# yinnhao/TAIR

Measured on AMD Instinct MI355X. Metric: restored Mpix/s @50-step SpacedSampler, 512² bf16; PSNR Δ vs ref ≤0.05 dB, higher is better.
Workload: dtype bf16; 1 GPU; configs[1]: 512x512 restoration, 50-step SpacedSampler, ControlLDM bf16, 1 tile(s)/GPU, hipGraph-replayed step, VAE decode included; tiles_per_gpu=1, micro_batch=1, global_batch=1, latent=64x64, sampling_steps=50, vae=HIP decoder, split-bf16 MFMA (fp32-accurate), parallelism=dp1 (tile-sharded replicas; RCCL all-gather of decoded tiles)

## Files before the change

### include/tair_kernels.h

```cpp
#ifndef TAIR_KERNELS_H
#define TAIR_KERNELS_H

#include <stdint.h>

#ifdef __cplusplus
extern "C" {
#endif

#define TAIR_A_DENSE 0
#define TAIR_A_CONV3 1
#define TAIR_A_CONV3_S2 2
#define TAIR_A_CONV3_UP 3
#define TAIR_A_CONV3_SMALLC 4

typedef struct {
  int M, N, K, amode;
  const void* A; int lda; int C; int Bn, H, W, Ho, Wo;
  const void* X; int ldx; int Kx;
  const void* Wt; int ldw;
  float alpha; int scale_bias; int act;
  const float* bias;
  const float* emb; int ld_emb; const int* emb_row; int rows_per_b;
  const void* res; int ld_res;
  void* out; int ldo; int out_f32;
  float* partial; int64_t partial_cap;
  int force_bm, force_bn, force_splits;
  int force_stages;
  int* tile_sem; int sem_cap;
  int out_split; int res_lo;
  double* st_acc; int st_rs, st_cg, st_G, st_coff, st_hw;
  int out_lo; int x_wrap;
  int probe;
  int f8; const float* row_scale; const float* col_scale;
  int s2_shift;
  const double* gn_st; int gn_rs; int gn_G; float gn_eps; const float* gn_gamma; const float* gn_beta; int gn_silu;
  unsigned long long* stamps;
  double* rst; const double* lnst; const float* lncs; float ln_c; float ln_eps;
} tair_gemm_desc;

int tair_k_gemm(const tair_gemm_desc* d, void* stream);
int tair_fault_count(int reset, int* count);
int tair_k_gemm_desc_bytes(void);
int tair_k_gemm_plan(const tair_gemm_desc* d, int* bm, int* bn, int* splits, int* kern);
int tair_k_attention_plan(int B, int H, int Sq, int Skv, int64_t ws_bytes, int* qsets, int* splits, int* kv_split);
int tair_k_attention(const void* q, int ldq, const void* k, int ldk, const void* v, int ldv, void* o, int ldo,
                     int B, int H, int Sq, int Skv, int kv_bstride, float scale, void* stream);
int tair_k_attention_ex(const void* q, int ldq, const void* k, int ldk, const void* v, int ldv, void* o, int ldo,
                        int B, int H, int Sq, int Skv, int kv_bstride, float scale, void* ws, int64_t ws_bytes,
                        int force_qsets, int force_splits, void* stream);
int tair_k_attention_tk(const void* q, int ldq, const void* k, int ldk, const void* v, int ldv, void* o, int ldo,
                        int B, int H, int Sq, int Skv, int kv_bstride, float scale, void* ws, int64_t ws_bytes,
                        int* tickets, int tickets_cap, int force_qsets, int force_splits, void* stream);
int tair_k_groupnorm(const void* x, int ldx, int B, int HW, int C, int G, float eps, const float* gamma,
                     const float* beta, int silu, void* y, int ldy, float* ss, float* ws, void* stream);
int tair_k_groupnorm_ex(const void* x, int ldx, int B, int HW, int C, int G, float eps, const float* gamma,
                        const float* beta, int silu, void* y, int ldy, float* ss, float* ws, int* tickets,
                        void* stream);
int tair_k_layernorm(const void* x, int T, int C, const float* gamma, const float* beta, float eps, void* y,
                     void* stream);
int tair_k_layernorm_fp8(const void* x, int T, int C, const float* gamma, const float* beta, float eps, void* y8,
                         int ld8, float* s8, void* stream);
int tair_k_quant_rows_fp8(const void* w, int rows, int K, int ldw, void* q, int ldq, float* scale, void* stream);
int tair_k_quant_rows_fp8_ex(const void* w, int rows, int K, int Kx, int ldw, const float* a, void* q, int ldq, int k8,
                             float* scale, void* stream);
int tair_k_gn_apply_fp8(const void* x, int ldx, int x_lo, int B, int HW, int C, int G, float eps, const float* gamma,
                        const float* beta, int silu, const double* st, int st_rs, const float* inv8, void* y8, int ld8,
// ... 34 lines not shown
```

### tair_amd/_lib.py

```python
from __future__ import annotations

import ctypes
import os
from typing import Optional

_HERE = os.path.dirname(os.path.abspath(__file__))
LIB_PATH = os.path.join(_HERE, "libtair_cldm.so")

TAIR_DTYPE_F32 = 0
TAIR_DTYPE_BF16 = 1
TAIR_DTYPE_FP8 = 2


class TairError(RuntimeError):
    pass


class CldmCfg(ctypes.Structure):
    _fields_ = [
        ("model_channels", ctypes.c_int),
        ("num_levels", ctypes.c_int),
        ("channel_mult", ctypes.c_int * 8),
        ("num_res_blocks", ctypes.c_int),
        ("num_attention_ds", ctypes.c_int),
# ... 86 lines not shown
    "tair_cldm_param_count": (_I, [_P, ctypes.POINTER(_I)]),
    "tair_cldm_param_info": (_I, [_P, _I, ctypes.POINTER(ctypes.c_char_p), ctypes.POINTER(ctypes.c_int64),
                                  ctypes.POINTER(_I)]),
    "tair_cldm_load_param": (_I, [_P, ctypes.c_char_p, _P, _I, ctypes.POINTER(ctypes.c_int64), _I]),
    "tair_cldm_finalize": (_I, [_P]),
    "tair_cldm_forward": (_I, [_P, ctypes.POINTER(CldmIO), _P]),
    "tair_sampler_set_schedule": (_I, [_P, _I, ctypes.POINTER(ctypes.c_int64), ctypes.POINTER(ctypes.c_float)]),
    "tair_sampler_prepare": (_I, [_P, ctypes.POINTER(SamplerIO), _P]),
    "tair_sampler_prepare_guided": (_I, [_P, ctypes.POINTER(SamplerIO), ctypes.POINTER(GuidanceIO), _P]),
    "tair_sampler_set_context": (_I, [_P, _P, _I, _P]),
    "tair_sampler_run": (_I, [_P, _I, _I, _P]),
    "tair_sampler_get_x": (_I, [_P, _P, _P, _P]),
    "tair_sampler_get_v": (_I, [_P, _P, _P]),
    "tair_profile_enable": (_I, [_P, _I]),
    "tair_profile_read": (_I, [_P, _I, ctypes.POINTER(ctypes.c_double), ctypes.POINTER(_I),
                               ctypes.POINTER(ctypes.c_double)]),
    "tair_cldm_flops": (_I, [_P, _I, ctypes.POINTER(ctypes.c_double)]),
    "tair_profile_dump": (_I, [_P, ctypes.c_char_p]),
    "tair_k_gemm": (_I, [ctypes.POINTER(GemmDesc), _P]),
    "tair_k_gemm_desc_bytes": (_I, []),
    "tair_fault_count": (_I, [_I, ctypes.POINTER(_I)]),
    "tair_k_gemm_plan": (_I, [ctypes.POINTER(GemmDesc), ctypes.POINTER(_I), ctypes.POINTER(_I), ctypes.POINTER(_I),
                              ctypes.POINTER(_I)]),
    "tair_k_attention_plan": (_I, [_I, _I, _I, _I, ctypes.c_int64, ctypes.POINTER(_I), ctypes.POINTER(_I),
                                   ctypes.POINTER(_I)]),
    "tair_k_attention": (_I, [_P, _I, _P, _I, _P, _I, _P, _I, _I, _I, _I, _I, _I, ctypes.c_float, _P]),
    "tair_k_attention_ex": (_I, [_P, _I, _P, _I, _P, _I, _P, _I, _I, _I, _I, _I, _I, ctypes.c_float, _P,
                                 ctypes.c_int64, _I, _I, _P]),
    "tair_k_attention_tk": (_I, [_P, _I, _P, _I, _P, _I, _P, _I, _I, _I, _I, _I, _I, ctypes.c_float, _P,
                                 ctypes.c_int64, _P, _I, _I, _I, _P]),
    "tair_k_groupnorm": (_I, [_P, _I, _I, _I, _I, _I, ctypes.c_float, _P, _P, _I, _P, _I, _P, _P, _P]),
    "tair_k_groupnorm_ex": (_I, [_P, _I, _I, _I, _I, _I, ctypes.c_float, _P, _P, _I, _P, _I, _P, _P, _P, _P]),
    "tair_k_layernorm": (_I, [_P, _I, _I, _P, _P, ctypes.c_float, _P, _P]),
    "tair_k_layernorm_fp8": (_I, [_P, _I, _I, _P, _P, ctypes.c_float, _P, _I, _P, _P]),
    "tair_k_quant_rows_fp8": (_I, [_P, _I, _I, _I, _P, _I, _P, _P]),
    "tair_k_geglu": (_I, [_P, _I, _I, _P, _P]),
    "tair_k_compose_ffpout": (_I, [_P, _P, _P, _P, _I, _P, _I, _P]),
    "tair_k_quant_rows_fp8_ex": (_I, [_P, _I, _I, _I, _I, _P, _P, _I, _I, _P, _P]),
    "tair_k_gn_apply_fp8": (_I, [_P, _I, _I, _I, _I, _I, _I, ctypes.c_float, _P, _P, _I, _P, _I, _P, _P, _I, _P]),
    "tair_k_sampler_step": (_I, [_P, _P, _P, _P, _P, _P, _P, _I, _I, _P, _P, _I, _I, _I, _P]),
    "tair_k_merge_overlap": (_I, [_P, _I, _I, _I, _I, _I, _I, _P, _I, _I, _I, _P, _P]),
    "tair_k_stitch_peers": (_I, [_P, _I, _I, _I, _I, _I, _I, _I, _I, _I, _I, _P, _I, _I, _I, _P, _P]),
    "tair_ipc_get_handle": (_I, [_P, _P, ctypes.POINTER(ctypes.c_ulonglong)]),
    "tair_ipc_open": (_I, [_P, ctypes.POINTER(ctypes.c_void_p)]),
    "tair_ipc_close": (_I, [_P]),
    "tair_k_gn_apply_stats": (_I, [_P, _I, _I, _I, _I, _I, _I, ctypes.c_float, _P, _P, _I, _P, _I, _P, _I, _I, _P]),
# ... 62 lines not shown
```

### tair_amd/csrc/gemm.hip

```cpp
#include <algorithm>

#include "gemm_kern.h"
#ifndef TAIR_BATCH_XCD
#define TAIR_BATCH_XCD 1
#endif

namespace tair {
namespace {

template <int S>
__global__ __launch_bounds__(256) void splitk_reduce_kernel(const GemmGroup P, int RB, int CB4) {
  const EpiArgs p = epi_args(P.g[blockIdx.z]);
  __shared__ double red[4 * STAT_NG];
  const int n4 = (p.N + 3) / 4;
  const size_t slab = (size_t)p.M * p.N;
  const bool vec = (p.N & 3) == 0;
  const bool stats = p.st[0].acc != nullptr;
  const int rpp = 256 / CB4;
  const int t = threadIdx.x;
  const int r0 = blockIdx.x * RB;
  const int c4_0 = blockIdx.y * CB4;
  if (stats) {
    for (int i = t; i < 4 * STAT_NG; i += 256) red[i] = 0.0;
    __syncthreads();
// ... 87 lines not shown
  TAIR_HIP_CHECK((gemm_set_attrs<A_DENSE, SET_SMALL>()));
  TAIR_HIP_CHECK((gemm_set_attrs<A_DENSE, SET_BIG>()));
  TAIR_HIP_CHECK((gemm_set_attrs<A_CONV3, SET_SMALL>()));
  TAIR_HIP_CHECK((gemm_set_attrs<A_CONV3, SET_BIG>()));
  TAIR_HIP_CHECK((gemm_set_attrs<A_CONV3_S2, SET_SMALL>()));
  TAIR_HIP_CHECK((gemm_set_attrs<A_CONV3_S2, SET_BIG>()));
  TAIR_HIP_CHECK((gemm_set_attrs<A_CONV3_UP, SET_SMALL>()));
  TAIR_HIP_CHECK((gemm_set_attrs<A_CONV3_UP, SET_BIG>()));
  TAIR_HIP_CHECK((gemm_set_attrs<A_CONV3_SMALLC, SET_REG>()));
  TAIR_HIP_CHECK((gemm_set_attrs<A_DENSE, SET_RING>()));
  TAIR_HIP_CHECK((gemm_set_attrs<A_CONV3, SET_RING>()));
  TAIR_HIP_CHECK((gemm_set_attrs<A_CONV3_S2, SET_RING>()));
  TAIR_HIP_CHECK((gemm_set_attrs<A_CONV3_UP, SET_RING>()));
  TAIR_HIP_CHECK((gemm_set_attrs<A_DENSE, SET_PHASE>()));
  TAIR_HIP_CHECK((gemm_set_attrs<A_DENSE, SET_SHALLOW>()));
  TAIR_HIP_CHECK((gemm_set_attrs<A_CONV3, SET_PHASE>()));
  TAIR_HIP_CHECK((gemm_set_attrs<A_CONV3_S2, SET_PHASE>()));
  TAIR_HIP_CHECK((gemm_set_attrs<A_CONV3_UP, SET_PHASE>()));
  TAIR_HIP_CHECK(set_attrs_f8<A_DENSE>());
  TAIR_HIP_CHECK((gemm_set_attrs<A_CONV3, SET_F8>()));
  TAIR_HIP_CHECK((gemm_set_attrs<A_CONV3, SET_HALO>()));
  TAIR_HIP_CHECK((gemm_set_attrs<A_DENSE, SET_DEEP>()));
  TAIR_HIP_CHECK((gemm_set_attrs<A_CONV3, SET_DEEP>()));
  done = true;
  return hipSuccess;
}

namespace {
hipError_t launch_set(int amode, GemmGroup& P, int n, int bm, int bn, int splits, int kern, hipStream_t s) {
  if (kern == GEMM_KERN_SHALLOW) return gemm_set_launch<A_DENSE, SET_SHALLOW>(P, n, bm, bn, splits, s);
  if (kern == GEMM_KERN_HALO) return gemm_set_launch<A_CONV3, SET_HALO>(P, n, bm, bn, splits, s);
  if (kern == GEMM_KERN_DEEP)
    return amode == A_DENSE ? gemm_set_launch<A_DENSE, SET_DEEP>(P, n, bm, bn, splits, s)
                            : gemm_set_launch<A_CONV3, SET_DEEP>(P, n, bm, bn, splits, s);
  if (kern == GEMM_KERN_PHASE) {
    switch (amode) {
      case A_DENSE: return gemm_set_launch<A_DENSE, SET_PHASE>(P, n, bm, bn, splits, s);
      case A_CONV3: return gemm_set_launch<A_CONV3, SET_PHASE>(P, n, bm, bn, splits, s);
      case A_CONV3_S2: return gemm_set_launch<A_CONV3_S2, SET_PHASE>(P, n, bm, bn, splits, s);
      default: return gemm_set_launch<A_CONV3_UP, SET_PHASE>(P, n, bm, bn, splits, s);
    }
  }
  if (bm < 0) {
    switch (amode) {
      case A_DENSE: return gemm_set_launch<A_DENSE, SET_RING>(P, n, -bm, bn, splits, s);
      case A_CONV3: return gemm_set_launch<A_CONV3, SET_RING>(P, n, -bm, bn, splits, s);
      case A_CONV3_S2: return gemm_set_launch<A_CONV3_S2, SET_RING>(P, n, -bm, bn, splits, s);
      default: return gemm_set_launch<A_CONV3_UP, SET_RING>(P, n, -bm, bn, splits, s);
    }
  }
  const bool big = gemm_tile_is_big(bm, bn);
  switch (amode) {
    case A_DENSE:
      return big ? gemm_set_launch<A_DENSE, SET_BIG>(P, n, bm, bn, splits, s)
                 : gemm_set_launch<A_DENSE, SET_SMALL>(P, n, bm, bn, splits, s);
    case A_CONV3:
      return big ? gemm_set_launch<A_CONV3, SET_BIG>(P, n, bm, bn, splits, s)
// ... 155 lines not shown
  *splits = s;
}

bool gemm_rowstats_ok(const GemmArgs& a) {
  static double probe_rst[2];
  GemmArgs b = a;
  if (!b.rst) b.rst = probe_rst;
  int bm, bn, s, kern;
  gemm_plan(b, &bm, &bn, &s, &kern);
  if (a.force_bm) bm = a.force_bm;
  return kern != GEMM_KERN_PHASE && (bm < 0 ? -bm : bm) <= 128 && !a.out_f32 && !a.out_split && a.act != 2 &&
         !a.st[0].acc;
}

size_t gemm_partial_elems(const GemmArgs& a) {
  int bm, bn, s;
  gemm_plan(a, &bm, &bn, &s);
  return s > 1 ? (size_t)s * a.M * a.N : 0;
}

static bool g_skip_reduce = false;
void gemm_set_skip_reduce(bool on) { g_skip_reduce = on; }

static int ink_smax() {
  static int v = -1;
  if (v < 0) {
    const char* e = getenv("TAIR_INK_SMAX");
    v = e ? atoi(e) : 3;
    if (v > INK_SMAX_BUILT) v = INK_SMAX_BUILT;
  }
  return v;
}

namespace {
thread_local bool g_gemm_dry = false;
thread_local int g_dry_plan[4];
thread_local bool g_gn_halo_only = false;
size_t plan_lds(int kern, int bm, int bn, int W, bool halo_s2) {
  if (kern == GEMM_KERN_HALO) {
    const int hrp = W == 64 ? (bn == 64 ? 448 : 400) : W == 32 ? (bn == 128 ? 384 : 344) : (bn == 128 ? 384 : 328);
    const int st = bn == 64 ? 4 : halo_s2 ? 2 : 3;
    return (size_t)2 * hrp * 128 + (size_t)st * bn * 128;
  }
  const int st = kern == GEMM_KERN_SHALLOW ? 2 : (bm == 128 && bn == 320) || (bm == 256 && bn >= 256) ? 2 : 3;
  return (size_t)st * (bm + bn) * 128;
}
bool deep_built(int bm, int bn, int st) {
  return bm == 64 && ((bn == 64 && (st == 4 || st == 5 || st == 6 || st == 8)) || (bn == 128 && st >= 4 && st <= 6));
}
}

bool gemm_gn_ok(const GemmArgs& a) {
  g_gemm_dry = g_gn_halo_only = true;
  const hipError_t e = gemm_grouped(&a, 1, nullptr);
  g_gemm_dry = g_gn_halo_only = false;
  return e == hipSuccess;
}

hipError_t gemm_plan_query(const GemmArgs& a, int* bm, int* bn, int* splits, int* kern, int lanes) {
  GemmArgs g[MAX_GROUP];
  const int n = lanes < 1 ? 1 : lanes > MAX_GROUP ? MAX_GROUP : lanes;
  for (int i = 0; i < n; ++i) g[i] = a;
  g_gemm_dry = true;
  const hipError_t e = gemm_grouped(g, n, nullptr);
  g_gemm_dry = false;
  *bm = g_dry_plan[0];
  *bn = g_dry_plan[1];
  *splits = g_dry_plan[2];
// ... 60 lines not shown
    return hipErrorInvalidValue;
  }
  if (a.lnst && (!a.lncs || a.amode != A_DENSE || a.Kx || a.f8 || !(a.ln_c > 0.f) || a.rst || a.st[0].acc ||
                 (a.N & 7))) {
    set_error("gemm: a folded LayerNorm takes a dense bf16 GEMM with column sums and 1/C");
    return hipErrorInvalidValue;
  }
  for (int i = 1; i < n; ++i)
    if ((args[i].rst != nullptr) != (a.rst != nullptr) || (args[i].lnst != nullptr) != (a.lnst != nullptr)) {
      set_error("gemm: grouped GEMMs must share the LayerNorm roles");
      return hipErrorInvalidValue;
    }
  int bm, bn, splits, kern;
  gemm_plan(a, &bm, &bn, &splits, &kern, n);
  if (a.force_bm) bm = a.force_bm;
  if (a.force_bn) bn = a.force_bn;
  if (a.force_splits) splits = a.force_splits;
  if (splits < 1 || splits > 16) {
    set_error("gemm: %d K splits (1..16)", splits);
    return hipErrorInvalidValue;
  }
  int tile_stages = 0;
  if (a.force_bm || a.force_stages)
    kern = a.force_stages >= 100 ? GEMM_KERN_DEEP
           : a.force_stages == 9 ? GEMM_KERN_HALO
           : a.force_stages >= 4 ? GEMM_KERN_PHASE : a.force_stages == 2 ? GEMM_KERN_SHALLOW : GEMM_KERN_TILE;
  if (kern == GEMM_KERN_DEEP) {
    tile_stages = a.force_stages - 100;
    if (a.f8 || (a.amode != A_DENSE && a.amode != A_CONV3) || !deep_built(bm, bn, tile_stages) || a.gn_st) {
      set_error("gemm: deep-ring tile %dx%d with %d stages not built (bf16 dense / stride-1 conv only)", bm, bn,
                tile_stages);
      return hipErrorInvalidValue;
    }
  }
  if (kern == GEMM_KERN_HALO && (!conv_halo_ok(a) || !halo_tile_built(a.W, bm, bn))) {
    set_error("gemm: halo tiles take bf16 stride-1 3x3 convs over 16/32/64-wide images, tile %dx%d not built "
              "for width %d", bm, bn, a.W);
    return hipErrorInvalidValue;
  }
  if (kern == GEMM_KERN_SHALLOW && (a.amode != A_DENSE || bm != 64 || (bn != 64 && bn != 128) || splits > 1)) {
    set_error("gemm: the 2-stage tiles are dense 64x64 / 64x128 without split-K (got %dx%d, mode %d, %d splits)", bm,
              bn, a.amode, splits);
    return hipErrorInvalidValue;
  }
  if (kern == GEMM_KERN_PHASE) splits = 1;
  if (kern == GEMM_KERN_PHASE && (a.amode == A_CONV3_SMALLC || bm != 256 || (bn != 256 && bn != 320))) {
    set_error("gemm: the 4-phase kernel takes 256x256 / 256x320 tiles (got %dx%d, mode %d)", bm, bn, a.amode);
    return hipErrorInvalidValue;
  }
  int st_hw = 0;
  for (int i = 0; i < n; ++i) {
    const GemmArgs& b = args[i];
    for (int k = 0; k < 2; ++k) {
      const StatTgt& t = b.st[k];
      if (!t.acc) continue;
      const bool groups_ok = t.cg >= 8 || (t.cg % 4 == 0 && t.c_off % 4 == 0);
// ... 47 lines not shown
      bm = 128;
      bn = a.amode == A_DENSE ? 256 : 320;
    }
    if (kern == GEMM_KERN_TILE && bm == 256 && bn != 128) bm = 128;
    if (kern == GEMM_KERN_TILE && bm == 128 && bn == 160) bn = 128;
    if (kern != GEMM_KERN_HALO)
      while (bm > 64 && a.rows_per_b % bm) bm >>= 1;
    const bool pipe_tile = kern == GEMM_KERN_SHALLOW || (bm == 128 && (bn == 256 || bn == 320)) ||
                           (bm == 256 && bn == 128);
    if (bm < 0 || (kern != GEMM_KERN_TILE && kern != GEMM_KERN_SHALLOW && kern != GEMM_KERN_HALO) ||
        (kern != GEMM_KERN_HALO && (a.rows_per_b % bm || !gemm_tile_built(a.amode, bm, bn) || !pipe_tile))) {
      set_error("gemm: no GroupNorm-on-load plan (tile %dx%d, kernel %d)", bm, bn, kern);
      return hipErrorInvalidValue;
    }
  }
  for (int i = 0; i < n; ++i) {
    const GemmArgs& b = args[i];
    while (splits > 1 && (b.partial == nullptr || (size_t)splits * b.M * b.N > b.partial_cap)) --splits;
  }
  {
    const int units = kern == GEMM_KERN_HALO ? a.C / 64 : (a.K + a.Kx) / (bm < 0 ? 32 : BK);
    while (splits > 1 && (long)(splits - 1) * cdiv(units, splits) >= units) --splits;
  }
  static const int b1_deep = [] { const char* e = getenv("TAIR_B1_DEEP"); return e ? atoi(e) : 0; }();
  if (b1_deep && kern == GEMM_KERN_TILE && !a.force_bm && !a.force_stages && !a.f8 && !a.gn_st && bm == 64 &&
      (bn == 64 || bn == 128) && (a.amode == A_DENSE || a.amode == A_CONV3)) {
    const long wgs = (long)cdiv(a.M, bm) * cdiv(a.N, bn) * splits * n;
    const int per = cdiv((a.K + a.Kx) / BK, splits);
    const long sb = (long)(bm + bn) * BK * 2;
    auto rounds = [&](int st) { const long slots = 256L * std::max(1L, (160L * 1024) / (st * sb)); return (wgs + slots - 1) / slots; };
    const long r0 = rounds(3);
    for (int st : {8, 6, 5, 4})
      if (st <= per + 1 && deep_built(bm, bn, st) && rounds(st) <= r0) {
        kern = GEMM_KERN_DEEP;
        tile_stages = st;
        break;
      }
  }
  static const bool coop_env = [] { const char* e = getenv("TAIR_COOP"); return !e || atoi(e) != 0; }();
  const bool coop_kind = coop_env && !g_skip_reduce && kern == GEMM_KERN_TILE && bm == 64 &&
                         a.amode != A_CONV3_SMALLC && !(a.probe & 4);
  if (a.rst && splits > 1)
    splits = ((kern == GEMM_KERN_TILE || kern == GEMM_KERN_DEEP) && bm == 64 && a.tile_sem)
                 ? (coop_kind ? splits : std::min(splits, std::max(1, ink_smax()))) : 1;
  if (a.amode < A_DENSE || a.amode > A_CONV3_SMALLC) {
    set_error("gemm: bad amode %d", a.amode);
    return hipErrorInvalidValue;
  }
  const bool f8_tile = (bm == 64 && (bn == 64 || bn == 128)) || (bm == 128 && (bn == 128 || bn == 256 || bn == 320));
  if (a.f8 && !f8_tile) {
    set_error("gemm: fp8 tile %dx%d not built", bm, bn);
    return hipErrorInvalidValue;
  }
  if (!a.f8 && kern != GEMM_KERN_PHASE && kern != GEMM_KERN_HALO &&
      (bm < 0 ? (a.amode == A_CONV3_SMALLC || !gemm_ring_built(-bm, bn) || (a.K % 32) || (a.Kx % 32))
              : !gemm_tile_built(a.amode, bm, bn))) {
    set_error("gemm: tile %dx%d not built for mode %d", bm, bn, a.amode);
    return hipErrorInvalidValue;
  }
  const int abm = bm < 0 ? -bm : bm;
  const long tiles_all = (long)cdiv(a.M, abm) * cdiv(a.N, bn);
  const long grid_wgs = tiles_all * splits * n;
  bool coop = splits > 1 && coop_kind && grid_wgs <= 2L * 256;
  for (int i = 0; i < n && coop; ++i)
    coop = args[i].tile_sem && tiles_all <= args[i].sem_cap &&
           (size_t)tiles_all * splits * abm * bn <= args[i].partial_cap;
  bool ink = splits > 1 && (coop || splits <= ink_smax() || (a.probe & 4)) && !g_skip_reduce &&
             a.amode != A_CONV3_SMALLC && (kern == GEMM_KERN_TILE || kern == GEMM_KERN_DEEP) &&
             bm == 64;
  for (int i = 0; i < n && ink; ++i)
    ink = args[i].tile_sem && tiles_all <= args[i].sem_cap &&
          (size_t)tiles_all * splits * abm * bn <= args[i].partial_cap;
  if (a.rst && splits > 1 && !ink) splits = 1;
  if (a.rst && (kern == GEMM_KERN_PHASE || (bm < 0 ? -bm : bm) > 128 || (splits > 1 && !ink))) {
    set_error("gemm: LayerNorm row statistics need a <= 128-row tile plan (got %dx%d, %d splits)", bm, bn, splits);
    return hipErrorInvalidValue;
  }
  GemmGroup P;
  P.fault = g_gemm_dry ? nullptr : fault_word();
  P.xcd = ((size_t)a.M * (a.K + a.Kx) * 2 > ((size_t)16 << 20) && a.N > (bn < 0 ? -bn : bn)) ? 2 : 1;
  {
    static const int xo = [] { const char* e = getenv("TAIR_XCD"); return e ? atoi(e) : 3; }();
    if (xo == 1 || xo == 2) P.xcd = xo;
    if (xo == 3 && a.N > (bn < 0 ? -bn : bn)) {
      const double ab = (double)a.M * (a.amode == A_DENSE ? a.K : a.C) * 2.0 + (double)a.M * a.Kx;
      const double wb = (double)a.N * (a.K + a.Kx) * 2.0;
      const long gx = cdiv(a.M, bm < 0 ? -bm : bm), gy = cdiv(a.N, bn);
      if (TAIR_BATCH_XCD && gx * gy * splits * n > 512) {
        const double nf = ab + wb * (double)std::min(8L, gx), mf = ab * (double)std::min(8L, gy) + wb;
        P.xcd = nf <= mf ? 2 : 1;
      } else if (ab > wb) {
// ... 31 lines not shown
          const double c = ab * (double)(gy / bnc) + wb * (double)(gx / bmr);
          if (c < 0.7 * best) {
            best = c;
            pick = 5 | (bmr << 8) | (bnc << 16);
          }
        }
      if (pick) P.xcd = pick;
    }
  }
  for (int i = n; i < MAX_GROUP; ++i) P.g[i] = P.g[0];

  if (a.gn_st && plan_lds(kern, bm, bn, a.W, P.g[0].halo_s2) + gn_extra_lds(P.g[0], splits) > 160 * 1024) {
    set_error("gemm: GroupNorm-on-load table does not fit the LDS (tile %dx%d, %d splits)", bm, bn, splits);
    return hipErrorInvalidValue;
  }
  if (g_gemm_dry) {
    g_dry_plan[0] = bm;
    g_dry_plan[1] = bn;
    g_dry_plan[2] = splits;
    g_dry_plan[3] = kern;
    if (g_gn_halo_only && a.gn_st && kern != GEMM_KERN_HALO) return hipErrorNotSupported;
    return hipSuccess;
  }
  hipError_t e = !a.f8 ? launch_set(a.amode, P, n, bm, bn, splits, kern, s)
                 : a.amode == A_DENSE ? launch_f8<A_DENSE>(P, n, bm, bn, splits, s, kern == GEMM_KERN_SHALLOW)
                                      : gemm_set_launch<A_CONV3, SET_F8>(P, n, bm, bn, splits, s);
  if (e != hipSuccess) return e;
  if (splits > 1 && !g_skip_reduce && !ink) {
    const int n4 = (a.N + 3) / 4;
    const int CB4 = n4 < 64 ? n4 : 64;
    const int cblocks = cdiv(n4, CB4);
    const int hw = st_hw ? st_hw : a.M;
    const int rpp = 256 / CB4;
    int RB = 1;
    while ((a.M % (RB * 2)) == 0 && (hw % (RB * 2)) == 0 && RB * 2 <= 4 * rpp &&
           (long)(a.M / (RB * 2)) * cblocks * n >= 256)
      RB *= 2;
    using RedFn = void (*)(const GemmGroup, int, int);
    static const RedFn red_fn[17] = {nullptr, nullptr,
                                     splitk_reduce_kernel<2>, splitk_reduce_kernel<3>, splitk_reduce_kernel<4>,
                                     splitk_reduce_kernel<5>, splitk_reduce_kernel<6>, splitk_reduce_kernel<7>,
                                     splitk_reduce_kernel<8>, splitk_reduce_kernel<9>, splitk_reduce_kernel<10>,
                                     splitk_reduce_kernel<11>, splitk_reduce_kernel<12>, splitk_reduce_kernel<13>,
                                     splitk_reduce_kernel<14>, splitk_reduce_kernel<15>, splitk_reduce_kernel<16>};
    hipLaunchKernelGGL(red_fn[splits], dim3(a.M / RB + (a.M % RB != 0), cblocks, n), dim3(256), 0, s, P, RB, CB4);
    e = hipGetLastError();
// ... 7 lines not shown
```

### tair_amd/csrc/gemm_kern.h

```cpp
#pragma once
#include <stdlib.h>

#include <type_traits>

#include "kernels.h"

namespace tair {

namespace {

__device__ __attribute__((aligned(1024))) uint4 g_zero_page[64];

constexpr int BK = 64;

template <class T>
TAIR_DEV const T& kernarg0() {
#if __HIP_DEVICE_COMPILE__
  return *(const T*)(const void*)__builtin_amdgcn_kernarg_segment_ptr();
#else
  return *(const T*)nullptr;
#endif
}

#ifndef TAIR_STAMPS
// ... 1752 lines not shown

  if constexpr (!F8 && (BM * BN >= 128 * 256 || (BM == 64 && STAGES >= 3))) {
    constexpr int CAP = STAGES * STAGE_BYTES;
    const EpiArgs ep = epi_args(p);
    switch (regstage_set<BM, BN, CAP>(ep)) {
#define TAIR_RS_CASE(S)                                                                 \
      case (S): epilogue_regstage<(S), BM, BN, FM, FN, WM, WN, NW * 64, CAP>(ep, acc, m0, n0, wm, wn, lane, smem); \
        return;
      TAIR_RS_CASE(E_BIAS | E_LNC | E_GEGLU)
      TAIR_RS_CASE(E_BIAS | E_GEGLU)
      TAIR_RS_CASE(E_BIAS | E_LNC)
      TAIR_RS_CASE(E_BIAS)
      TAIR_RS_CASE(E_BIAS | E_ROWST)
      TAIR_RS_CASE(E_BIAS | E_RES | E_ROWST)
      TAIR_RS_CASE(E_BIAS | E_RES)
#undef TAIR_RS_CASE
      default: break;
    }
  }
  epilogue_tile<BM, BN, FM, FN, WM, WN, NW * 64, STAGES * STAGE_BYTES, (BM == 64 && STAGES >= 3),
                !(BM == 64 && STAGES == 2)>(p, acc, m0, n0, wm, wn, lane, smem, bz);
}

template <int S, int GW, int WX, int GH, int HX>
TAIR_DEV void halo_wait(int wid, bool pend) {
  const bool wf = WX == 0 || wid < WX, hx = HX != 0 && wid < HX;
  if (pend) {
    if (wf) {
      if (hx) wait_vmcnt<(S - 2) * GW + GH + 1>();
      else wait_vmcnt<(S - 2) * GW + GH>();
    } else {
      if (hx) wait_vmcnt<(S - 2) * (GW - 1) + GH + 1>();
      else wait_vmcnt<(S - 2) * (GW - 1) + GH>();
    }
  } else {
    if (wf) wait_vmcnt<(S - 2) * GW>();
    else wait_vmcnt<(S - 2) * (GW - 1)>();
  }
}

template <int BN, int HRP, int STAGES, int ABL = 0>
__global__ __launch_bounds__(512) void conv_halo_kernel(const GemmGroup P_arg) {
  constexpr int BM = 256, WMW = 4, WNW = 2, NW = 8;
  constexpr int WM = BM / WMW, WN = BN / WNW;
  constexpr int FM = WM / 16, FN = WN / 16;
  constexpr int GW = (BN + 8 * NW - 1) / (8 * NW);
// ... 658 lines not shown
  TAIR_HIP_CHECK((set_attr_tile<T64x64D4, AMODE>()));
  TAIR_HIP_CHECK((set_attr_tile<T64x64D5, AMODE>()));
  TAIR_HIP_CHECK((set_attr_tile<T64x64D6, AMODE>()));
  TAIR_HIP_CHECK((set_attr_tile<T64x64D8, AMODE>()));
  TAIR_HIP_CHECK((set_attr_tile<T64x128D4, AMODE>()));
  TAIR_HIP_CHECK((set_attr_tile<T64x128D5, AMODE>()));
  TAIR_HIP_CHECK((set_attr_tile<T64x128D6, AMODE>()));
  return hipSuccess;
}
template <int AMODE>
hipError_t launch_deep(GemmGroup& a, int n, int bm, int bn, int splits, hipStream_t s) {
  const int st = a.g[0].tile_stages;
  if (bm == 64 && bn == 64) {
    if (st == 4) return launch_tile<T64x64D4, AMODE>(a, n, splits, s);
    if (st == 5) return launch_tile<T64x64D5, AMODE>(a, n, splits, s);
    if (st == 6) return launch_tile<T64x64D6, AMODE>(a, n, splits, s);
    if (st == 8) return launch_tile<T64x64D8, AMODE>(a, n, splits, s);
  }
  if (bm == 64 && bn == 128) {
    if (st == 4) return launch_tile<T64x128D4, AMODE>(a, n, splits, s);
    if (st == 5) return launch_tile<T64x128D5, AMODE>(a, n, splits, s);
    if (st == 6) return launch_tile<T64x128D6, AMODE>(a, n, splits, s);
  }
  return hipErrorInvalidValue;
}
template <int AMODE>
hipError_t set_attrs_big() {
  TAIR_HIP_CHECK((set_attr_tile<T128x256, AMODE>()));
  TAIR_HIP_CHECK((set_attr_tile<T256x256, AMODE>()));
  TAIR_HIP_CHECK((set_attr_tile<T128x320, AMODE>()));
  TAIR_HIP_CHECK((set_attr_tile<T256x320, AMODE>()));
  TAIR_HIP_CHECK((set_attr_tile<T256x160, AMODE>()));
  TAIR_HIP_CHECK((set_attr_tile<T256x128, AMODE>()));
  return hipSuccess;
}
template <int AMODE>
hipError_t launch_big(GemmGroup& a, int n, int bm, int bn, int splits, hipStream_t s) {
  if (bm == 128 && bn == 256) return launch_tile<T128x256, AMODE>(a, n, splits, s);
  if (bm == 256 && bn == 256) return launch_tile<T256x256, AMODE>(a, n, splits, s);
  if (bm == 128 && bn == 320) return launch_tile<T128x320, AMODE>(a, n, splits, s);
  if (bm == 256 && bn == 320) return launch_tile<T256x320, AMODE>(a, n, splits, s);
  if (bm == 256 && bn == 160) return launch_tile<T256x160, AMODE>(a, n, splits, s);
  if (bm == 256 && bn == 128) return launch_tile<T256x128, AMODE>(a, n, splits, s);
  return hipErrorInvalidValue;
}

// ... 159 lines not shown
hipError_t launch_phase_tile(GemmGroup& a, int n, int splits, hipStream_t s) {
  a.tiles_m = cdiv(a.g[0].M, 256);
  dim3 grid(a.tiles_m * n, cdiv(a.g[0].N, BN), splits);
  hipLaunchKernelGGL((gemm_phase_kernel<BN, AMODE, ABL>), grid, dim3(512), PhaseCfg<BN>::LDS, s, a);
  return hipGetLastError();
}
template <int AMODE>
hipError_t launch_phase(GemmGroup& a, int n, int bm, int bn, int splits, hipStream_t s) {
  if constexpr (AMODE == A_CONV3) {
    if (a.g[0].force_stages == 5 && bn == 256) return launch_phase_tile<256, AMODE, 1>(a, n, splits, s);
    if (a.g[0].force_stages == 6 && bn == 256) return launch_phase_tile<256, AMODE, 2>(a, n, splits, s);
  }
  if (bm != 256) return hipErrorInvalidValue;
  if (bn == 256) return launch_phase_tile<256, AMODE>(a, n, splits, s);
  if (bn == 320) return launch_phase_tile<320, AMODE>(a, n, splits, s);
  return hipErrorInvalidValue;
}

}

template <int AMODE, int SET> hipError_t gemm_set_attrs();
template <int AMODE, int SET> hipError_t gemm_set_launch(GemmGroup& a, int n, int bm, int bn, int splits, hipStream_t s);
constexpr int SET_SMALL = 0, SET_BIG = 1, SET_REG = 2, SET_RING = 3, SET_PHASE = 4, SET_SHALLOW = 5, SET_F8 = 6,
              SET_HALO = 7, SET_DEEP = 8;

}

#define TAIR_GEMM_SET_TU(AMODE, SET, KIND)                                                             \
  namespace tair {                                                                                     \
  template <>                                                                                          \
  hipError_t gemm_set_attrs<AMODE, SET>() {                                                            \
    return set_attrs_##KIND<AMODE>();                                                                  \
  }                                                                                                    \
  template <>                                                                                          \
  hipError_t gemm_set_launch<AMODE, SET>(GemmGroup & a, int n, int bm, int bn, int splits, hipStream_t s) { \
    return launch_##KIND<AMODE>(a, n, bm, bn, splits, s);                                              \
  }                                                                                                    \
  }
```

### tair_amd/csrc/kapi.cpp

```cpp
#include <cstring>
#include "kernels.h"
#include "tair_kernels.h"

using namespace tair;

extern "C" {

namespace {
GemmArgs gemm_args_of(const tair_gemm_desc* d) {
  GemmArgs a{};
  a.M = d->M; a.N = d->N; a.K = d->K; a.amode = d->amode;
  a.A = (const bf16*)d->A; a.lda = d->lda; a.C = d->C;
  a.Bn = d->Bn; a.H = d->H; a.W = d->W; a.Ho = d->Ho; a.Wo = d->Wo;
  a.X = (const bf16*)d->X; a.ldx = d->ldx; a.Kx = d->Kx;
  a.Wt = (const bf16*)d->Wt; a.ldw = d->ldw;
  a.alpha = d->alpha; a.scale_bias = d->scale_bias; a.act = d->act;
  a.bias = d->bias;
  a.emb = d->emb; a.ld_emb = d->ld_emb; a.emb_row = d->emb_row; a.rows_per_b = d->rows_per_b > 0 ? d->rows_per_b : 1;
  a.res = (const bf16*)d->res; a.ld_res = d->ld_res;
  a.out = d->out; a.ldo = d->ldo; a.out_f32 = d->out_f32;
  a.splits = 1; a.partial = d->partial; a.partial_cap = (size_t)d->partial_cap;
  a.force_bm = d->force_bm; a.force_bn = d->force_bn; a.force_splits = d->force_splits;
  a.force_stages = d->force_stages;
  a.tile_sem = d->tile_sem; a.sem_cap = d->sem_cap;
// ... 24 lines not shown
  return gemm(a, (hipStream_t)stream) == hipSuccess ? 0 : -2;
}

int tair_fault_count(int reset, int* count) {
  if (!count) return -1;
  return gemm_fault_count(count, reset != 0) == hipSuccess ? 0 : -2;
}

int tair_k_gemm_desc_bytes(void) { return (int)sizeof(tair_gemm_desc); }

int tair_k_compose_ffpout(const float* wpout, const float* wff2, const float* bff2, const float* bpout, int C,
                          void* packed, int ldp, float* bias) {
  if (!wpout || !wff2 || !bff2 || !bpout || !packed || !bias || C < 1 || ldp < 5 * C) return -1;
  compose_ffpout(wpout, wff2, bff2, bpout, C, (uint16_t*)packed, ldp, bias);
  return 0;
}

int tair_k_gemm_plan(const tair_gemm_desc* d, int* bm, int* bn, int* splits, int* kern) {
  if (!d || !bm || !bn || !splits || !kern) return -1;
  const GemmArgs a = gemm_args_of(d);
  return gemm_plan_query(a, bm, bn, splits, kern) == hipSuccess ? 0 : -2;
}

int tair_k_attention_plan(int B, int H, int Sq, int Skv, int64_t ws_bytes, int* qsets, int* splits, int* kv_split) {
  if (!qsets || !splits || !kv_split || B < 1 || H < 1 || Sq < 1 || Skv < 1) return -1;
  const AttnPlan p = attention_plan(B, H, Sq, Skv, ws_bytes < 0 ? (size_t)-1 : (size_t)ws_bytes);
  *qsets = p.qsets;
  *splits = p.splits;
  *kv_split = p.kv_split;
  return 0;
}

int tair_k_attention(const void* q, int ldq, const void* k, int ldk, const void* v, int ldv, void* o, int ldo,
                     int B, int H, int Sq, int Skv, int kv_bstride, float scale, void* stream) {
  return attention((const bf16*)q, ldq, (const bf16*)k, ldk, (const bf16*)v, ldv, (bf16*)o, ldo, B, H, Sq, Skv,
                   kv_bstride, scale, (hipStream_t)stream) == hipSuccess ? 0 : -2;
}

int tair_k_attention_ex(const void* q, int ldq, const void* k, int ldk, const void* v, int ldv, void* o, int ldo,
                        int B, int H, int Sq, int Skv, int kv_bstride, float scale, void* ws, int64_t ws_bytes,
                        int force_qsets, int force_splits, void* stream) {
  return attention((const bf16*)q, ldq, (const bf16*)k, ldk, (const bf16*)v, ldv, (bf16*)o, ldo, B, H, Sq, Skv,
                   kv_bstride, scale, (hipStream_t)stream, ws, ws ? (size_t)ws_bytes : 0, force_qsets,
                   force_splits) == hipSuccess ? 0 : -2;
}

// ... 174 lines not shown
```

### tair_amd/csrc/kernels.h

```cpp
#pragma once
#include "common.h"

namespace tair {

enum AMode : int {
  A_DENSE = 0,
  A_CONV3 = 1,
  A_CONV3_S2 = 2,
  A_CONV3_UP = 3,
  A_CONV3_SMALLC = 4,
};

constexpr int STAT_REPL = 8;
struct StatTgt {
  double* acc;
  int rs;
  int cg, G;
  int c_off;
  int hw;
};

struct GemmArgs {
  int M, N, K;
  int amode;
// ... 43 lines not shown
  GemmArgs g[MAX_GROUP];
  int tiles_m;
  int xcd;
  int* fault;
};


inline bool gemm_tile_built(int amode, int bm, int bn) {
  if (amode == A_CONV3_SMALLC) return bm == 64 && (bn == 64 || bn == 128);
  const bool small = (bm == 64 || bm == 128) && (bn == 64 || bn == 128);
  const bool big = (bm == 128 && (bn == 256 || bn == 320)) ||
                   (bm == 256 && (bn == 128 || bn == 160 || bn == 256 || bn == 320));
  return small || big;
}
inline bool gemm_tile_is_big(int bm, int bn) { return bn > 128 || bm > 128; }
constexpr bool gemm_tile_pipe(int waves, int stages) { return waves == 8 || stages == 2; }
inline bool gemm_ring_built(int bm, int bn) {
  return (bm == 128 && (bn == 320 || bn == 256 || bn == 128)) || (bm == 256 && (bn == 256 || bn == 128)) ||
         (bm == 64 && (bn == 128 || bn == 64));
}

hipError_t gemm(const GemmArgs& a, hipStream_t s);
void gemm_set_skip_reduce(bool on);
constexpr int GEMM_TICKETS = 16384;
constexpr int ATTN_TICKETS = 16384;
hipError_t gemm_grouped(const GemmArgs* a, int n, hipStream_t s);
bool gemm_gn_ok(const GemmArgs& a);
hipError_t gemm_plan_query(const GemmArgs& a, int* bm, int* bn, int* splits, int* kern, int lanes = 1);
hipError_t gemm_init();
hipError_t gemm_fault_count(int* count, bool reset);
constexpr int GEMM_KERN_TILE = 0, GEMM_KERN_PHASE = 1, GEMM_KERN_SHALLOW = 2;
constexpr int GEMM_KERN_HALO = 3;
constexpr int GEMM_KERN_DEEP = 4;
bool conv_halo_ok(const GemmArgs& a);
void gemm_plan(const GemmArgs& a, int* bm, int* bn, int* splits, int* kern = nullptr, int lanes = 1);
size_t gemm_partial_elems(const GemmArgs& a);
bool gemm_rowstats_ok(const GemmArgs& a);

hipError_t groupnorm_scale_shift(const bf16* x, int ldx, int B, int HW, int C, int G, float eps,
                                 const float* gamma, const float* beta, float* scale_shift,
                                 float* ws, hipStream_t s, int* tickets = nullptr);
struct GnArgs {
  const bf16* x; int ldx;
  const float* gamma; const float* beta;
  float* ss;
  float* ws;
  int* tickets;
  bf16* y; int ldy;
  const double* st; int st_rs; float eps;
  int x_lo; int y_split;
  uint8_t* y8 = nullptr; int ld8 = 0; const float* inv8 = nullptr;
};
struct GnGroup { GnArgs g[MAX_GROUP]; };
hipError_t groupnorm_stats_grouped(const GnArgs* a, int n, int B, int HW, int C, int G, float eps,
                                   hipStream_t s);
hipError_t groupnorm_apply_grouped(const GnArgs* a, int n, int B, int HW, int C, int silu, hipStream_t s,
// ... 81 lines not shown
```

Measured before the change: 1.030 Mpix/s.

## Add two-K-group GEMM kernel splitting K within a workgroup for conv3 tiles

```diff
diff --git a/include/tair_kernels.h b/include/tair_kernels.h
--- a/include/tair_kernels.h
+++ b/include/tair_kernels.h
@@ -42,6 +42,9 @@
 int tair_fault_count(int reset, int* count);
 int tair_k_gemm_desc_bytes(void);
 int tair_k_gemm_plan(const tair_gemm_desc* d, int* bm, int* bn, int* splits, int* kern);
+int tair_k_kgroup_trips(int kt0, int kt1);
+int tair_k_gemm_kgroup_force(int on);
+int tair_k_kgroup_tile(int kt0, int g, int trip);
 int tair_k_attention_plan(int B, int H, int Sq, int Skv, int64_t ws_bytes, int* qsets, int* splits, int* kv_split);
 int tair_k_attention(const void* q, int ldq, const void* k, int ldk, const void* v, int ldv, void* o, int ldo,
                      int B, int H, int Sq, int Skv, int kv_bstride, float scale, void* stream);
diff --git a/tair_amd/_lib.py b/tair_amd/_lib.py
--- a/tair_amd/_lib.py
+++ b/tair_amd/_lib.py
@@ -132,6 +132,9 @@
     "tair_fault_count": (_I, [_I, ctypes.POINTER(_I)]),
     "tair_k_gemm_plan": (_I, [ctypes.POINTER(GemmDesc), ctypes.POINTER(_I), ctypes.POINTER(_I), ctypes.POINTER(_I),
                               ctypes.POINTER(_I)]),
+    "tair_k_kgroup_trips": (_I, [_I, _I]),
+    "tair_k_gemm_kgroup_force": (_I, [_I]),
+    "tair_k_kgroup_tile": (_I, [_I, _I, _I]),
     "tair_k_attention_plan": (_I, [_I, _I, _I, _I, ctypes.c_int64, ctypes.POINTER(_I), ctypes.POINTER(_I),
                                    ctypes.POINTER(_I)]),
     "tair_k_attention": (_I, [_P, _I, _P, _I, _P, _I, _P, _I, _I, _I, _I, _I, _I, ctypes.c_float, _P]),
diff --git a/tair_amd/csrc/gemm.hip b/tair_amd/csrc/gemm.hip
--- a/tair_amd/csrc/gemm.hip
+++ b/tair_amd/csrc/gemm.hip
@@ -133,6 +133,8 @@
   TAIR_HIP_CHECK((gemm_set_attrs<A_CONV3, SET_HALO>()));
   TAIR_HIP_CHECK((gemm_set_attrs<A_DENSE, SET_DEEP>()));
   TAIR_HIP_CHECK((gemm_set_attrs<A_CONV3, SET_DEEP>()));
+  TAIR_HIP_CHECK((gemm_set_attrs<A_DENSE, SET_KGROUP>()));
+  TAIR_HIP_CHECK((gemm_set_attrs<A_CONV3, SET_KGROUP>()));
   done = true;
   return hipSuccess;
 }
@@ -144,6 +146,9 @@
   if (kern == GEMM_KERN_DEEP)
     return amode == A_DENSE ? gemm_set_launch<A_DENSE, SET_DEEP>(P, n, bm, bn, splits, s)
                             : gemm_set_launch<A_CONV3, SET_DEEP>(P, n, bm, bn, splits, s);
+  if (kern == GEMM_KERN_KGROUP)
+    return amode == A_DENSE ? gemm_set_launch<A_DENSE, SET_KGROUP>(P, n, bm, bn, splits, s)
+                            : gemm_set_launch<A_CONV3, SET_KGROUP>(P, n, bm, bn, splits, s);
   if (kern == GEMM_KERN_PHASE) {
     switch (amode) {
       case A_DENSE: return gemm_set_launch<A_DENSE, SET_PHASE>(P, n, bm, bn, splits, s);
@@ -345,6 +350,15 @@
 static bool g_skip_reduce = false;
 void gemm_set_skip_reduce(bool on) { g_skip_reduce = on; }
 
+static bool g_kgroup_force = false;
+static long g_kgroup_launches = 0;
+long gemm_set_kgroup_force(bool on) {
+  g_kgroup_force = on;
+  const long c = g_kgroup_launches;
+  g_kgroup_launches = 0;
+  return c;
+}
+
 static int ink_smax() {
   static int v = -1;
   if (v < 0) {
@@ -367,6 +381,18 @@
   }
   const int st = kern == GEMM_KERN_SHALLOW ? 2 : (bm == 128 && bn == 320) || (bm == 256 && bn >= 256) ? 2 : 3;
   return (size_t)st * (bm + bn) * 128;
+}
+int kgroup_rule(const GemmArgs& a, int bm, int bn, int splits, int lanes) {
+  const int ktiles = (a.K + a.Kx) / BK;
+  const long tiles = (long)cdiv(a.M, bm) * cdiv(a.N, bn) * lanes;
+  if (a.amode != A_CONV3 || a.Bn != 1 || !a.tile_sem) return 0;
+  if (tiles * splits > 512 || tiles > 256 || tiles < 32) return 0;
+  int s2 = std::min((int)(256 / tiles), ktiles / 15);
+  s2 = std::max(1, std::min(s2, splits));
+  while (s2 > 1 && (long)(s2 - 1) * cdiv(ktiles, s2) >= ktiles) --s2;
+  if (ktiles / s2 < 4) return 0;
+  if (s2 == 1 && splits > 1 && ktiles > 100) return 0;
+  return s2;
 }
 bool deep_built(int bm, int bn, int st) {
   return bm == 64 && ((bn == 64 && (st == 4 || st == 5 || st == 6 || st == 8)) || (bn == 128 && st >= 4 && st <= 6));
@@ -473,7 +499,8 @@
   }
   int tile_stages = 0;
   if (a.force_bm || a.force_stages)
-    kern = a.force_stages >= 100 ? GEMM_KERN_DEEP
+    kern = a.force_stages >= 200 ? GEMM_KERN_KGROUP
+           : a.force_stages >= 100 ? GEMM_KERN_DEEP
            : a.force_stages == 9 ? GEMM_KERN_HALO
            : a.force_stages >= 4 ? GEMM_KERN_PHASE : a.force_stages == 2 ? GEMM_KERN_SHALLOW : GEMM_KERN_TILE;
   if (kern == GEMM_KERN_DEEP) {
@@ -483,6 +510,12 @@
                 tile_stages);
       return hipErrorInvalidValue;
     }
+  }
+  if (kern == GEMM_KERN_KGROUP &&
+      (a.f8 || a.gn_st || !gemm_kgroup_built(a.amode, bm, bn, a.force_stages - 200))) {
+    set_error("gemm: two-K-group tile %dx%d with %d stages not built (bf16 dense / stride-1 conv, 64x64 / 64x128, "
+              "3 stages, no GroupNorm on load; mode %d, fp8 %d)", bm, bn, a.force_stages - 200, a.amode, a.f8);
+    return hipErrorInvalidValue;
   }
   if (kern == GEMM_KERN_HALO && (!conv_halo_ok(a) || !halo_tile_built(a.W, bm, bn))) {
     set_error("gemm: halo tiles take bf16 stride-1 3x3 convs over 16/32/64-wide images, tile %dx%d not built "
@@ -576,6 +609,21 @@
     const int units = kern == GEMM_KERN_HALO ? a.C / 64 : (a.K + a.Kx) / (bm < 0 ? 32 : BK);
     while (splits > 1 && (long)(splits - 1) * cdiv(units, splits) >= units) --splits;
   }
+#ifndef TAIR_NO_KGROUP
+  if (kern == GEMM_KERN_TILE && !a.force_bm && !a.force_bn && !a.force_splits && !a.force_stages && !a.f8 &&
+      !a.gn_st && gemm_kgroup_built(a.amode, bm, bn, 3)) {
+    int s2 = kgroup_rule(a, bm, bn, splits, n);
+    if (g_kgroup_force) {
+      const int units = (a.K + a.Kx) / BK;
+      s2 = cdiv(splits, 2);
+      while (s2 > 1 && (long)(s2 - 1) * cdiv(units, s2) >= units) --s2;
+    }
+    if (s2) {
+      kern = GEMM_KERN_KGROUP;
+      splits = s2;
+    }
+  }
+#endif
   static const int b1_deep = [] { const char* e = getenv("TAIR_B1_DEEP"); return e ? atoi(e) : 0; }();
   if (b1_deep && kern == GEMM_KERN_TILE && !a.force_bm && !a.force_stages && !a.f8 && !a.gn_st && bm == 64 &&
       (bn == 64 || bn == 128) && (a.amode == A_DENSE || a.amode == A_CONV3)) {
@@ -592,10 +640,10 @@
       }
   }
   static const bool coop_env = [] { const char* e = getenv("TAIR_COOP"); return !e || atoi(e) != 0; }();
-  const bool coop_kind = coop_env && !g_skip_reduce && kern == GEMM_KERN_TILE && bm == 64 &&
+  const bool coop_kind = coop_env && !g_skip_reduce && (kern == GEMM_KERN_TILE || kern == GEMM_KERN_KGROUP) && bm == 64 &&
                          a.amode != A_CONV3_SMALLC && !(a.probe & 4);
   if (a.rst && splits > 1)
-    splits = ((kern == GEMM_KERN_TILE || kern == GEMM_KERN_DEEP) && bm == 64 && a.tile_sem)
+    splits = ((kern == GEMM_KERN_TILE || kern == GEMM_KERN_DEEP || kern == GEMM_KERN_KGROUP) && bm == 64 && a.tile_sem)
                  ? (coop_kind ? splits : std::min(splits, std::max(1, ink_smax()))) : 1;
   if (a.amode < A_DENSE || a.amode > A_CONV3_SMALLC) {
     set_error("gemm: bad amode %d", a.amode);
@@ -615,12 +663,13 @@
   const int abm = bm < 0 ? -bm : bm;
   const long tiles_all = (long)cdiv(a.M, abm) * cdiv(a.N, bn);
   const long grid_wgs = tiles_all * splits * n;
-  bool coop = splits > 1 && coop_kind && grid_wgs <= 2L * 256;
+  bool coop = splits > 1 && coop_kind && grid_wgs <= (kern == GEMM_KERN_KGROUP ? 256 : 2L * 256);
   for (int i = 0; i < n && coop; ++i)
     coop = args[i].tile_sem && tiles_all <= args[i].sem_cap &&
            (size_t)tiles_all * splits * abm * bn <= args[i].partial_cap;
   bool ink = splits > 1 && (coop || splits <= ink_smax() || (a.probe & 4)) && !g_skip_reduce &&
-             a.amode != A_CONV3_SMALLC && (kern == GEMM_KERN_TILE || kern == GEMM_KERN_DEEP) &&
+             a.amode != A_CONV3_SMALLC &&
+             (kern == GEMM_KERN_TILE || kern == GEMM_KERN_DEEP || kern == GEMM_KERN_KGROUP) &&
              bm == 64;
   for (int i = 0; i < n && ink; ++i)
     ink = args[i].tile_sem && tiles_all <= args[i].sem_cap &&
@@ -698,6 +747,7 @@
     if (g_gn_halo_only && a.gn_st && kern != GEMM_KERN_HALO) return hipErrorNotSupported;
     return hipSuccess;
   }
+  if (kern == GEMM_KERN_KGROUP) ++g_kgroup_launches;
   hipError_t e = !a.f8 ? launch_set(a.amode, P, n, bm, bn, splits, kern, s)
                  : a.amode == A_DENSE ? launch_f8<A_DENSE>(P, n, bm, bn, splits, s, kern == GEMM_KERN_SHALLOW)
                                       : gemm_set_launch<A_CONV3, SET_F8>(P, n, bm, bn, splits, s);
diff --git a/tair_amd/csrc/gemm_conv3_kgroup.hip b/tair_amd/csrc/gemm_conv3_kgroup.hip
--- /dev/null
+++ b/tair_amd/csrc/gemm_conv3_kgroup.hip
@@ -0,0 +1,3 @@
+#include "gemm_kern.h"
+
+TAIR_GEMM_SET_TU(A_CONV3, SET_KGROUP, kgroup)
diff --git a/tair_amd/csrc/gemm_dense_kgroup.hip b/tair_amd/csrc/gemm_dense_kgroup.hip
--- /dev/null
+++ b/tair_amd/csrc/gemm_dense_kgroup.hip
@@ -0,0 +1,3 @@
+#include "gemm_kern.h"
+
+TAIR_GEMM_SET_TU(A_DENSE, SET_KGROUP, kgroup)
diff --git a/tair_amd/csrc/gemm_kern.h b/tair_amd/csrc/gemm_kern.h
--- a/tair_amd/csrc/gemm_kern.h
+++ b/tair_amd/csrc/gemm_kern.h
@@ -1798,6 +1798,169 @@
                 !(BM == 64 && STAGES == 2)>(p, acc, m0, n0, wm, wn, lane, smem, bz);
 }
 
+template <int BM, int BN, int AMODE>
+__global__ __launch_bounds__(512) void gemm_kgroup_kernel(const GemmGroup P_arg) {
+  constexpr int WMW = 2, WNW = 2, NW = 4, STAGES = 3;
+  constexpr int WM = BM / WMW, WN = BN / WNW;
+  constexpr int FM = WM / 16, FN = WN / 16;
+  constexpr int NA = BM / (8 * NW), NB = BN / (8 * NW);
+  constexpr int G = NA + NB;
+  constexpr int STAGE_BYTES = (BM + BN) * BK * 2;
+  constexpr int RING = STAGES * STAGE_BYTES;
+  static_assert(BM == 64 && (BN == 64 || BN == 128), "two-K-group tiles: 64x64 / 64x128");
+  static_assert(2 * RING <= 160 * 1024 && NW * FM * FN * 1024 <= RING, "LDS");
+  extern __shared__ __attribute__((aligned(16))) char smem[];
+
+  const GemmGroup& P = kernarg0<GemmGroup>();
+  int xcd = P.xcd, tiles_m = P.tiles_m;
+  TAIR_PIN_ASM("" : "+s"(xcd), "+s"(tiles_m));
+  int bxl, by, bz;
+  xcd_remap(bxl, by, bz, xcd);
+  const int grp = bxl / tiles_m;
+  const int bx = bxl - grp * tiles_m;
+  const GemmArgs& p = P.g[grp];
+  stamp(p, 0);
+  const MainArgs ma = main_args(p);
+
+  const int tid = threadIdx.x, lane = tid & 63;
+  const int wid8 = __builtin_amdgcn_readfirstlane(tid >> 6);
+  const int kg = wid8 >> 2, wid = wid8 & 3;
+  const int wm = wid % WMW, wn = wid / WMW;
+  const int m0 = bx * BM, n0 = by * BN;
+  const int ktot = (ma.K + ma.Kx) / BK;
+  const int per = (ktot + ma.splits - 1) / ma.splits;
+  const int kt0 = bz * per;
+  const int kt1 = min(ktot, kt0 + per);
+  const int trips = kgroup_trips(kt0, kt1);
+
+  const int drow = lane >> 3;
+  const int dchunk = (lane & 7) ^ drow;
+  RowInfo<AMODE> rows[NA];
+#pragma unroll
+  for (int i = 0; i < NA; ++i) rows[i] = row_info<AMODE>(ma, m0 + (i * NW + wid) * 8 + drow, dchunk);
+  const bf16* wrow[NB];
+#pragma unroll
+  for (int i = 0; i < NB; ++i) {
+    const int n = n0 + (i * NW + wid) * 8 + drow;
+    wrow[i] = n < ma.N ? ma.Wt + (size_t)n * ma.ldw + dchunk * 8 : nullptr;
+  }
+  const bf16* zp = (const bf16*)g_zero_page;
+  const ActArgs pa = act_args(ma);
+
+  f32x4 acc[FN][FM];
+#pragma unroll
+  for (int j = 0; j < FN; ++j)
+#pragma unroll
+    for (int i = 0; i < FM; ++i) acc[j][i] = f32x4{0.f, 0.f, 0.f, 0.f};
+
+  char* const ring = smem + kg * RING;
+#define TAIR_KG_ISSUE(KT, STG)                                                                    \
+  do {                                                                                            \
+    const int k0_ = (KT) * BK;                                                                    \
+    char* sb_ = ring + (STG) * STAGE_BYTES;                                                       \
+    _Pragma("unroll") for (int i = 0; i < NA; ++i)                                                \
+      __builtin_amdgcn_global_load_lds((const void*)act_src<AMODE>(pa, rows[i], k0_),             \
+                                       TAIR_LDS(sb_ + (i * NW + wid) * 8 * 128), 16, 0, 0);       \
+    _Pragma("unroll") for (int i = 0; i < NB; ++i)                                                \
+      __builtin_amdgcn_global_load_lds((const void*)(wrow[i] ? wrow[i] + k0_ : zp),              \
+                                       TAIR_LDS(sb_ + BM * 128 + (i * NW + wid) * 8 * 128), 16, 0, 0); \
+  } while (0)
+
+  const uint32_t lds0 = lds_u32(ring);
+  const int ra = wm * WM + (lane & 15), rb = wn * WN + (lane & 15);
+  const uint32_t aoff0 = ra * 128 + ((((lane >> 4)) ^ (ra & 7)) << 4);
+  const uint32_t aoff1 = ra * 128 + (((4 + (lane >> 4)) ^ (ra & 7)) << 4);
+  const uint32_t boff0 = BM * 128 + rb * 128 + ((((lane >> 4)) ^ (rb & 7)) << 4);
+  const uint32_t boff1 = BM * 128 + rb * 128 + (((4 + (lane >> 4)) ^ (rb & 7)) << 4);
+
+  if (trips > 0) {
+    const int kl = kt1 - 1;
+#pragma unroll
+    for (int s = 0; s < STAGES - 1; ++s) TAIR_KG_ISSUE(min(kgroup_tile(kt0, kg, s), kl), s);
+    stamp(p, 1);
+    int stage = 0;
+    for (int j = 0; j < trips; ++j) {
+      const int t = kgroup_tile(kt0, kg, j);
+      wait_vmcnt<(STAGES - 2) * G>();
+      __builtin_amdgcn_s_barrier();
+      if (j == 0) stamp(p, 2);
+      int ps = stage + STAGES - 1;
+      if (ps >= STAGES) ps -= STAGES;
+      TAIR_KG_ISSUE(min(kgroup_tile(kt0, kg, j + STAGES - 1), kl), ps);
+      if (t < kt1) {
+        const uint32_t sb = lds0 + stage * STAGE_BYTES;
+        bf16x8 xf[FM], wf[FN];
+        ds_read_frags<FM>(xf, sb + aoff0);
+        ds_read_frags<FN>(wf, sb + boff0);
+        wait_lgkmcnt<0>();
+        touch<FM>(xf);
+        touch<FN>(wf);
+        __builtin_amdgcn_sched_barrier(0);
+#pragma unroll
+        for (int jj = 0; jj < FN; ++jj)
+#pragma unroll
+          for (int i = 0; i < FM; ++i)
+            acc[jj][i] = __builtin_amdgcn_mfma_f32_16x16x32_bf16(wf[jj], xf[i], acc[jj][i], 0, 0, 0);
+        __builtin_amdgcn_sched_barrier(0);
+        ds_read_frags<FM>(xf, sb + aoff1);
+        ds_read_frags<FN>(wf, sb + boff1);
+        wait_lgkmcnt<0>();
+        touch<FM>(xf);
+        touch<FN>(wf);
+        __builtin_amdgcn_sched_barrier(0);
+#pragma unroll
+        for (int jj = 0; jj < FN; ++jj)
+#pragma unroll
+          for (int i = 0; i < FM; ++i)
+            acc[jj][i] = __builtin_amdgcn_mfma_f32_16x16x32_bf16(wf[jj], xf[i], acc[jj][i], 0, 0, 0);
+      }
+      stage = (stage + 1 == STAGES) ? 0 : stage + 1;
+    }
+    wait_vmcnt<0>();
+    stamp(p, 3);
+  }
+#undef TAIR_KG_ISSUE
+
+  __syncthreads();
+  if (kg == 1) {
+    static_for<0, FN>([&](auto J) {
+      constexpr int j = decltype(J)::value;
+      static_for<0, FM>([&](auto I) {
+        constexpr int i = decltype(I)::value;
+        *(f32x4*)(smem + (((wid * FN + j) * FM + i) * 64 + lane) * 16) = acc[j][i];
+      });
+    });
+  }
+  __syncthreads();
+  if (kg == 1) return;
+  static_for<0, FN>([&](auto J) {
+    constexpr int j = decltype(J)::value;
+    static_for<0, FM>([&](auto I) {
+      constexpr int i = decltype(I)::value;
+      acc[j][i] = acc[j][i] + *(const f32x4*)(smem + (((wid * FN + j) * FM + i) * 64 + lane) * 16);
+    });
+  });
+
+  {
+    const EpiArgs ep = epi_args(p);
+    switch (regstage_set<BM, BN, RING>(ep)) {
+#define TAIR_RS_CASE(S)                                                                 \
+      case (S): epilogue_regstage<(S), BM, BN, FM, FN, WM, WN, NW * 64, RING>(ep, acc, m0, n0, wm, wn, lane, smem); \
+        return;
+      TAIR_RS_CASE(E_BIAS | E_LNC | E_GEGLU)
+      TAIR_RS_CASE(E_BIAS | E_GEGLU)
+      TAIR_RS_CASE(E_BIAS | E_LNC)
+      TAIR_RS_CASE(E_BIAS)
+      TAIR_RS_CASE(E_BIAS | E_ROWST)
+      TAIR_RS_CASE(E_BIAS | E_RES | E_ROWST)
+      TAIR_RS_CASE(E_BIAS | E_RES)
+#undef TAIR_RS_CASE
+      default: break;
+    }
+  }
+  epilogue_tile<BM, BN, FM, FN, WM, WN, NW * 64, RING, true, true>(p, acc, m0, n0, wm, wn, lane, smem, bz);
+}
+
 template <int S, int GW, int WX, int GH, int HX>
 TAIR_DEV void halo_wait(int wid, bool pend) {
   const bool wf = WX == 0 || wid < WX, hx = HX != 0 && wid < HX;
@@ -2502,6 +2665,33 @@
     if (st == 5) return launch_tile<T64x128D5, AMODE>(a, n, splits, s);
     if (st == 6) return launch_tile<T64x128D6, AMODE>(a, n, splits, s);
   }
+  return hipErrorInvalidValue;
+}
+template <int BN, int AMODE>
+hipError_t launch_kgroup_tile(GemmGroup& a, int n, int splits, hipStream_t s) {
+  constexpr size_t LDS = 2 * T64x64::STAGES * (size_t)(64 + BN) * BK * sizeof(bf16);
+  a.tiles_m = cdiv(a.g[0].M, 64);
+  dim3 grid(a.tiles_m * n, cdiv(a.g[0].N, BN), splits);
+  if (a.g[0].coop) {
+    const long cap = resident_wgs(gemm_kgroup_kernel<64, BN, AMODE>, 512, LDS);
+    if ((long)grid.x * grid.y * grid.z > cap)
+      for (int i = 0; i < MAX_GROUP; ++i) a.g[i].coop = 0;
+  }
+  hipLaunchKernelGGL((gemm_kgroup_kernel<64, BN, AMODE>), grid, dim3(512), LDS, s, a);
+  return hipGetLastError();
+}
+template <int AMODE>
+hipError_t set_attrs_kgroup() {
+  TAIR_HIP_CHECK(hipFuncSetAttribute((const void*)gemm_kgroup_kernel<64, 64, AMODE>,
+                                     hipFuncAttributeMaxDynamicSharedMemorySize, 160 * 1024));
+  TAIR_HIP_CHECK(hipFuncSetAttribute((const void*)gemm_kgroup_kernel<64, 128, AMODE>,
+                                     hipFuncAttributeMaxDynamicSharedMemorySize, 160 * 1024));
+  return hipSuccess;
+}
+template <int AMODE>
+hipError_t launch_kgroup(GemmGroup& a, int n, int bm, int bn, int splits, hipStream_t s) {
+  if (bm == 64 && bn == 64) return launch_kgroup_tile<64, AMODE>(a, n, splits, s);
+  if (bm == 64 && bn == 128) return launch_kgroup_tile<128, AMODE>(a, n, splits, s);
   return hipErrorInvalidValue;
 }
 template <int AMODE>
@@ -2707,7 +2897,7 @@
 template <int AMODE, int SET> hipError_t gemm_set_attrs();
 template <int AMODE, int SET> hipError_t gemm_set_launch(GemmGroup& a, int n, int bm, int bn, int splits, hipStream_t s);
 constexpr int SET_SMALL = 0, SET_BIG = 1, SET_REG = 2, SET_RING = 3, SET_PHASE = 4, SET_SHALLOW = 5, SET_F8 = 6,
-              SET_HALO = 7, SET_DEEP = 8;
+              SET_HALO = 7, SET_DEEP = 8, SET_KGROUP = 9;
 
 }
 
diff --git a/tair_amd/csrc/kapi.cpp b/tair_amd/csrc/kapi.cpp
--- a/tair_amd/csrc/kapi.cpp
+++ b/tair_amd/csrc/kapi.cpp
@@ -70,6 +70,10 @@
   return gemm_plan_query(a, bm, bn, splits, kern) == hipSuccess ? 0 : -2;
 }
 
+int tair_k_gemm_kgroup_force(int on) { return (int)gemm_set_kgroup_force(on != 0); }
+int tair_k_kgroup_trips(int kt0, int kt1) { return kgroup_trips(kt0, kt1); }
+int tair_k_kgroup_tile(int kt0, int g, int trip) { return kgroup_tile(kt0, g, trip); }
+
 int tair_k_attention_plan(int B, int H, int Sq, int Skv, int64_t ws_bytes, int* qsets, int* splits, int* kv_split) {
   if (!qsets || !splits || !kv_split || B < 1 || H < 1 || Sq < 1 || Skv < 1) return -1;
   const AttnPlan p = attention_plan(B, H, Sq, Skv, ws_bytes < 0 ? (size_t)-1 : (size_t)ws_bytes);
diff --git a/tair_amd/csrc/kernels.h b/tair_amd/csrc/kernels.h
--- a/tair_amd/csrc/kernels.h
+++ b/tair_amd/csrc/kernels.h
@@ -89,6 +89,7 @@
 
 hipError_t gemm(const GemmArgs& a, hipStream_t s);
 void gemm_set_skip_reduce(bool on);
+long gemm_set_kgroup_force(bool on);
 constexpr int GEMM_TICKETS = 16384;
 constexpr int ATTN_TICKETS = 16384;
 hipError_t gemm_grouped(const GemmArgs* a, int n, hipStream_t s);
@@ -99,6 +100,12 @@
 constexpr int GEMM_KERN_TILE = 0, GEMM_KERN_PHASE = 1, GEMM_KERN_SHALLOW = 2;
 constexpr int GEMM_KERN_HALO = 3;
 constexpr int GEMM_KERN_DEEP = 4;
+constexpr int GEMM_KERN_KGROUP = 5;
+inline bool gemm_kgroup_built(int amode, int bm, int bn, int stages) {
+  return (amode == A_DENSE || amode == A_CONV3) && bm == 64 && (bn == 64 || bn == 128) && stages == 3;
+}
+__host__ __device__ inline int kgroup_trips(int kt0, int kt1) { return kt1 > kt0 ? (kt1 - kt0 + 1) / 2 : 0; }
+__host__ __device__ inline int kgroup_tile(int kt0, int g, int trip) { return kt0 + g + 2 * trip; }
 bool conv_halo_ok(const GemmArgs& a);
 void gemm_plan(const GemmArgs& a, int* bm, int* bn, int* splits, int* kern = nullptr, int lanes = 1);
 size_t gemm_partial_elems(const GemmArgs& a);
```

Result: faster. 1.057 Mpix/s (median of 6 runs) (+2.6%).
